# fpthink/PDGN

Hardware: AMD Instinct MI355X
Metric: generator+D step points/sec (B=35, 256->2048 pts) (higher is better)
Workload: dtype f32; 1 GPU; PDGNet_v2 G+D iteration (models/PDGNet_v2.py:171-256), chair-shaped synthetic batch, per-GPU batch 35, 256->2048 pts, random-init weights; global_batch=35, parallelism=dp1, losses_finite=True, hipgraph=False, issue=list

## Files before the change

### pdgn_amd/csrc/gemm_rp.hip

```cpp
#include "gemm_shared.h"

typedef _Float16 rp_f16x8 __attribute__((ext_vector_type(8)));
typedef _Float16 rp_f16x2 __attribute__((ext_vector_type(2)));
typedef float rp_f32x16 __attribute__((ext_vector_type(16)));
typedef float rp_f32x2 __attribute__((ext_vector_type(2)));

struct RpArgs {
    long long M;
    int N, lda, ldw, ldc;
    const float *A;
    const unsigned short *Wp;
    long long wplane;
    float *C;
    const unsigned *max_w;
    int panels, ctiles;
    int rgroups, cslabs;
    int wg_per_xcd;
    float *stat_part;
};

__device__ __forceinline__ unsigned rp_cvt_pk(float a, float b) {
    const rp_f32x2 v = {a, b};
    return __builtin_bit_cast(unsigned, __builtin_convertvector(v, rp_f16x2));
}
__device__ __forceinline__ rp_f32x16 rp_mfma(const u32x4 a, const u32x4 b, const rp_f32x16 c) {
    return __builtin_amdgcn_mfma_f32_32x32x16_f16(__builtin_bit_cast(rp_f16x8, a), __builtin_bit_cast(rp_f16x8, b), c, 0, 0, 0);
}
__device__ __forceinline__ unsigned rp_sw(unsigned r) { return (r >> 2) & 3u; }

template <int K, int AUX, bool PIPE, bool STATS = false>
__global__ __launch_bounds__(512, 1) void gemm_rp_kernel(const RpArgs p) {
    static_assert(K == 32 || K == 64 || K == 128, "reduction lengths of the per-point products");
    constexpr int KS = K / 16, KC = K / 32;
    constexpr int BN = 64, BM = 256;
    constexpr int PLANE = KC * BN * 64;
    constexpr int WTILE = 2 * PLANE;
    constexpr int STL = STATS ? 2 * (8 * 3 * BN + 8) * 4 : 0;
    __shared__ __attribute__((aligned(1024))) unsigned char smem[2 * WTILE + 2 * BN * 4 + 8 * 4096 + STL];
    int *const colexp = reinterpret_cast<int *>(smem + 2 * WTILE);
    float *const stl = reinterpret_cast<float *>(smem + 2 * WTILE + 2 * BN * 4 + 8 * 4096);
    const int tid = threadIdx.x, lane = tid & 63;
    const int wave = __builtin_amdgcn_readfirstlane(tid >> 6);
    unsigned char *const stg = smem + 2 * WTILE + 2 * BN * 4 + wave * 4096;
    const int li = lane & 31, lg = lane >> 5;

    const int xcd = blockIdx.x & 7, slot = blockIdx.x >> 3;
    const int rgi = xcd / p.cslabs, csi = xcd - rgi * p.cslabs;
    const int ppg = (p.panels + p.rgroups - 1) / p.rgroups, cps = (p.ctiles + p.cslabs - 1) / p.cslabs;
    const int p0 = rgi * ppg, p1 = min(p.panels, p0 + ppg);
    const int c0 = csi * cps, c1 = min(p.ctiles, c0 + cps);
    if (p0 >= p1 || c0 >= c1) return;
    const int nc = c1 - c0;
    const long long steps = (long long)(p1 - p0) * nc;
    long long t = steps * slot / p.wg_per_xcd;
    const long long t1 = steps * (slot + 1) / p.wg_per_xcd;
    if (t >= t1) return;

    constexpr int PIECES = 2 * BN * (K / 8) / 512;
    static_assert(PIECES >= 1, "a weight tile is at least one piece per thread");
    u32x4 wraw[PIECES];
    int craw = 0;
    const __amdgpu_buffer_rsrc_t rsW = __builtin_amdgcn_make_buffer_rsrc((void *)p.Wp, 0, (int)min((2 * p.wplane) * 2LL, 0x7fffffffLL), 0x00020000);
    const __amdgpu_buffer_rsrc_t rsMW = __builtin_amdgcn_make_buffer_rsrc((void *)p.max_w, 0, p.N * 4, 0x00020000);
    auto load_w = [&](int ct) {
        const int n0 = (c0 + ct) * BN;
#pragma unroll
        for (int j = 0; j < PIECES; ++j) {
            const int id = tid + 512 * j;
            const int part = id / (BN * (K / 8)), rem = id - part * (BN * (K / 8));
            const int row = rem / (K / 8), c = rem - row * (K / 8);
            const bool ok = ct < nc && n0 + row < p.N;
            const unsigned off = (unsigned)(((long long)part * p.wplane + (long long)(n0 + row) * p.ldw + 8 * c) * 2);
            wraw[j] = __builtin_bit_cast(u32x4, __builtin_amdgcn_raw_buffer_load_b128(rsW, ok ? off : NT_OOB, 0, 0));
        }
        if (tid < BN) craw = __builtin_amdgcn_raw_buffer_load_b32(rsMW, (ct < nc && n0 + tid < p.N) ? (unsigned)(n0 + tid) * 4u : NT_OOB, 0, 0);
    };
    auto write_w = [&](int buf) {
#pragma unroll
        for (int j = 0; j < PIECES; ++j) {
            const int id = tid + 512 * j;
            const int part = id / (BN * (K / 8)), rem = id - part * (BN * (K / 8));
            const int row = rem / (K / 8), c = rem - row * (K / 8);
            *reinterpret_cast<u32x4 *>(smem + buf * WTILE + part * PLANE + (c >> 2) * (BN * 64) + row * 64 + (((c & 3) ^ rp_sw(row)) * 16)) = wraw[j];
        }
        if (tid < BN) colexp[buf * BN + tid] = 127 - x2_scale_field((unsigned)craw);
    };

    u32x4 afh[KS], afl[KS];
    int ua_e[4];
    int cur_mrows = 0;
    __amdgpu_buffer_rsrc_t rsC = __builtin_amdgcn_make_buffer_rsrc((void *)p.C, 0, 0, 0x00020000);
    auto load_a = [&](int panel) {
        const long long m0 = (long long)panel * BM + 32 * wave;
        const int mrows = (int)max(0LL, min(32LL, p.M - m0));
        cur_mrows = mrows;
        const __amdgpu_buffer_rsrc_t rsA = __builtin_amdgcn_make_buffer_rsrc((void *)(p.A + m0 * p.lda), 0,
                                                                            mrows > 0 ? (int)(((long long)(mrows - 1) * p.lda + K) * 4) : 0, 0x00020000);
        f32x4 raw[2 * KS];
#pragma unroll
        for (int s = 0; s < KS; ++s) {
            const unsigned off = li < mrows ? (unsigned)(li * p.lda + 16 * s + 8 * lg) * 4u : NT_OOB;
            raw[2 * s] = __builtin_bit_cast(f32x4, __builtin_amdgcn_raw_buffer_load_b128(rsA, off, 0, 0));
            raw[2 * s + 1] = __builtin_bit_cast(f32x4, __builtin_amdgcn_raw_buffer_load_b128(rsA, off == NT_OOB ? NT_OOB : off + 16u, 0, 0));
        }
        unsigned mb = 0u;
#pragma unroll
        for (int i = 0; i < 2 * KS; ++i)
#pragma unroll
            for (int r = 0; r < 4; ++r) mb = max(mb, __float_as_uint(raw[i][r]) & 0x7fffffffu);
        mb = max(mb, (unsigned)__shfl_xor((int)mb, 32));
        const int f = x2_scale_field(mb);
        const float sc = __int_as_float(f << 23);
#pragma unroll
// ... 171 lines not shown
#pragma unroll
            for (int part = 0; part < 4; ++part) out_part(prev, part);
        }
        const bool more = t + 1 < t1;
        const int nct = next_ct(ct);
        if (more) write_w(buf ^ 1);
        const bool more2 = t + 2 < t1;
        if (more2) load_w(next_ct(nct));
        if (more && nct == 0) {
            ++panel;
            load_a(panel);
        }
        ct = nct;
        buf ^= 1;
        asm volatile("s_waitcnt lgkmcnt(0)" ::: "memory");
        __builtin_amdgcn_s_barrier();
        asm volatile("" ::: "memory");
    }
    if (STATS && comb) stat_combine(comb_panel, comb_n0, comb_sb);
    if (PIPE && have_prev) {
#pragma unroll
        for (int part = 0; part < 4; ++part) out_part(prev, part);
    }
    if (STATS && have_prev) {
        asm volatile("s_waitcnt lgkmcnt(0)" ::: "memory");
        __builtin_amdgcn_s_barrier();
        asm volatile("" ::: "memory");
        stat_combine(prev_panel, prev.n0, prev.sbuf);
    }
}

template <int K>
static void rp_go(int grid, hipStream_t s, const RpArgs &a, int aux, bool pipe) {
    if (a.stat_part) {
        if (aux == 2) hipLaunchKernelGGL((gemm_rp_kernel<K, 2, true, true>), dim3(grid), dim3(512), 0, s, a);
        else hipLaunchKernelGGL((gemm_rp_kernel<K, 0, true, true>), dim3(grid), dim3(512), 0, s, a);
    } else if (!pipe) hipLaunchKernelGGL((gemm_rp_kernel<K, 2, false>), dim3(grid), dim3(512), 0, s, a);
    else if (aux == 16) hipLaunchKernelGGL((gemm_rp_kernel<K, 16, true>), dim3(grid), dim3(512), 0, s, a);
    else if (aux == 2) hipLaunchKernelGGL((gemm_rp_kernel<K, 2, true>), dim3(grid), dim3(512), 0, s, a);
    else hipLaunchKernelGGL((gemm_rp_kernel<K, 0, true>), dim3(grid), dim3(512), 0, s, a);
}

bool rp_takes(long long m, int n, int k) {
    static const bool off = [] { const char *e = getenv("PDGN_RP"); return e && e[0] == '0'; }();
    return !off && (k == 32 || k == 64 || k == 128) && n >= 128 && m >= 4096 && (double)m * n >= 1.6e7 && m < (1LL << 28);
}

int rp_launch(long long m, int n, int k, const float *A, int lda, const unsigned short *Wp, int ldw, long long wplane, float *C, int ldc,
              float *stat_part, hipStream_t s) {
    RpArgs a;
    a.stat_part = stat_part;
    a.M = m; a.N = n; a.lda = lda; a.ldw = ldw; a.ldc = ldc; a.A = A; a.Wp = Wp; a.wplane = wplane; a.C = C;
    a.max_w = reinterpret_cast<const unsigned *>(Wp + 2 * wplane);
    a.panels = cdiv(m, 256);
    a.ctiles = cdiv(n, 64);
    static const int force_cs = [] { const char *e = getenv("PDGN_RP_CSLABS"); return e ? atoi(e) : 0; }();
    int cs = 1;
    while (cs < 8 && (double)cdiv(a.ctiles, cs) * 64 * k * 4 > 2.0e6) cs *= 2;
    if (force_cs == 1 || force_cs == 2 || force_cs == 4 || force_cs == 8) cs = force_cs;
    while (cs > 1 && (a.ctiles < cs || a.panels < 8 / cs)) cs /= 2;
    a.cslabs = cs;
    a.rgroups = 8 / cs;
    const int cus = nt_cus();
    a.wg_per_xcd = cus >= 8 ? cus / 8 : 1;
    static const int aux_env = [] { const char *e = getenv("PDGN_RP_STORE"); return e ? atoi(e) : -1; }();
    const int aux = aux_env >= 0 ? aux_env : ((double)m * n * 4 > 2.5e8 ? 2 : 0);
    static const bool pipe = [] { const char *e = getenv("PDGN_RP_PIPE"); return !(e && e[0] == '0'); }();
    const int grid = 8 * a.wg_per_xcd;
    if (k == 128) rp_go<128>(grid, s, a, aux, pipe);
    else if (k == 64) rp_go<64>(grid, s, a, aux, pipe);
    else rp_go<32>(grid, s, a, aux, pipe);
    return pdgn_launch_status();
}
```

### pdgn_amd/csrc/gemm_x3.hip

```cpp
#include <atomic>
#include <type_traits>

#include "gemm_shared.h"

#ifndef X3_FENCE
#define X3_FENCE 2
#endif
#ifndef X3_DEFAULT_MASK
#define X3_DEFAULT_MASK 0x000
#endif
#ifndef X3_FENCE16
#define X3_FENCE16 2
#endif
#ifndef X3_ABLATE
#define X3_ABLATE 0
#endif

typedef float f32x16 __attribute__((ext_vector_type(16)));
typedef float f32x2 __attribute__((ext_vector_type(2)));
typedef __bf16 bf16x8 __attribute__((ext_vector_type(8)));
typedef __bf16 bf16x2 __attribute__((ext_vector_type(2)));

struct X3Parts {
    u32x4 h, m, l;
// ... 1051 lines not shown
        const unsigned long long at = next.fetch_add(need);
        const unsigned long long pos = at % slots;
        if (pos + need <= slots) return ring + (size_t)pos * 256;
    }
}
const unsigned *x2_scan(const float *X, long long rows, int cols, int ld, bool bycol, hipStream_t s) {
    unsigned *out = x2_arena_take(bycol ? cols : rows);
    if (!out) return nullptr;
    if (x2_maxima_launch(X, rows, cols, ld, bycol ? nullptr : out, bycol ? out : nullptr, s) != 0) return nullptr;
    return out;
}
static thread_local const unsigned *x2_next_max_a = nullptr, *x2_next_max_w = nullptr;

static thread_local const unsigned *x2_cur_max_a = nullptr, *x2_cur_max_w = nullptr;
struct X3Handover {
    X3Handover() {
        x3_cur_ws = x3_tail_ws; x3_cur_ws_floats = x3_tail_ws_floats;
        x2_cur_max_a = x2_next_max_a; x2_cur_max_w = x2_next_max_w;
        x3_tail_ws = nullptr; x3_tail_ws_floats = 0;
        x2_next_max_a = x2_next_max_w = nullptr;
    }
    ~X3Handover() {
        x3_cur_ws = nullptr; x3_cur_ws_floats = 0;
        x2_cur_max_a = x2_cur_max_w = nullptr;
    }
};

static int x3_reduce_split(int tiles) {
    int y = 8;
    while (tiles * y < 512 && y < 64) y *= 2;
    return y;
}

bool rp_takes(long long m, int n, int k);
int rp_launch(long long m, int n, int k, const float *A, int lda, const unsigned short *Wp, int ldw, long long wplane, float *C, int ldc,
              float *stat_part, hipStream_t s);
void x3_launch16(int cfg, int flags, int grid, hipStream_t s, const NtArgs &a);
void x3_launch_h2(int flags, int grid, hipStream_t s, const NtArgs &a, bool eight_waves);
const void *x3_symbol_h2(int flags, bool eight_waves);
static bool x2_pays(int cfg, long long m, int n, int k, long long scan_bytes) {
    if (nt_switches().mode != 2 || cfg != 0 || k < 128 || m >= (1LL << 28)) return false;
    const double flops = 2.0 * (double)m * n * k;
    static const double min_flops = [] { const char *e = getenv("PDGN_X2_MIN_GFLOP"); return (e && *e) ? atof(e) * 1e9 : 2e10; }();
    return flops >= min_flops && (double)scan_bytes <= 4.5e-3 * flops;
}

template <int TM, int TN, int WM, int WN, int OCC, int RATE, int CFG>
struct X3Cfg {
    static constexpr int BM = 32 * TM * WM, BN = 32 * TN * WN;
    static constexpr int LDS = 2 * 3 * (BM + BN) * 64;
    static constexpr int WG_PER_CU = OCC;

    struct Plan {
        int tiles_m, tiles_n, kchunks, grid_dp, dp_tiles, grid_sk;
        long long sk_per_wg;
        double cost;
    };
    static int dp_grid(long long tiles, int slots, int kc) {
        int tpw = (64 + kc - 1) / kc;
        tpw = tpw < 1 ? 1 : (tpw > 8 ? 8 : tpw);
        const long long g = (tiles + tpw - 1) / tpw;
        const long long lo = tiles < slots ? tiles : slots;
        return (int)(g < lo ? lo : g);
    }
    static double chunk_us(int w) { return 2.0 * BM * BN * NT_BK * w / (RATE * 1e3); }
    static Plan plan(long long m, int n, int k, bool allow_sk) {
        Plan pl;
// ... 303 lines not shown

extern "C" int pdgn_gemm_nt_ex(long long m, int n, int k, const float *A, int lda, const float *W, int ldw, const float *bias,
                               const float *addend, int ldadd, float *C, int ldc, float *stat_part, const float *row_bias,
                               int ld_rb, int rows_per_group, int act, const float *gate, int ldgate, int transposed_w,
                               pdgn_stream_t stream) {
    const X3Handover handover;
    if (!x3_mode())
        return fp32_gemm_nt_ex(m, n, k, A, lda, W, ldw, bias, addend, ldadd, C, ldc, stat_part, row_bias, ld_rb, rows_per_group,
                               act, gate, ldgate, transposed_w, stream);
    if (!x3_args_ok(m, n, k, lda, ldw, ldadd, ldc, addend, transposed_w != 0)) return PDGN_ERR_INVALID;
    if ((act != 0 && act != 2) || (row_bias && (ld_rb < n || ld_rb % 4 || rows_per_group < 1)) ||
        (gate && (ldgate < n || ldgate % 4)) || m >= (1LL << 31) || (row_bias && m * rows_per_group >= (1LL << 32)) ||
        (row_bias && rows_per_group >= 1 && ((m + rows_per_group - 1) / rows_per_group) * (long long)ld_rb * 4 >= (long long)NT_OOB))
        return PDGN_ERR_INVALID;
    NtEpi e;
    e.row_bias = row_bias; e.ld_rb = ld_rb; e.rows_per_group = rows_per_group; e.act = act; e.gate = gate; e.ldgate = ldgate;
    return transposed_w ? x3_dispatch<true>(m, n, k, A, lda, W, ldw, bias, addend, ldadd, C, ldc, stat_part, (hipStream_t)stream, e)
                        : x3_dispatch<false>(m, n, k, A, lda, W, ldw, bias, addend, ldadd, C, ldc, stat_part, (hipStream_t)stream, e);
}

extern "C" int pdgn_gemm_nt_ps(long long m, int n, int k, const float *A, int lda, const unsigned short *Wplanes, int ldw,
                               long long wplane, int parts, const float *bias, const float *addend, int ldadd, float *C, int ldc,
                               float *stat_part, const float *row_bias, int ld_rb, int rows_per_group, int act, const float *gate,
                               int ldgate, pdgn_stream_t stream) {
    const X3Handover handover;
    if (!x3_mode() || !Wplanes || (parts != 3 && parts != 2)) return PDGN_ERR_INVALID;
    if (!x3_args_ok(m, n, k, lda, ldw, ldadd, ldc, addend, false)) return PDGN_ERR_INVALID;
    if (wplane < (long long)(n - 1) * ldw + k || wplane >= (1LL << 28) || ldw % 8 || wplane % 8 || ((uintptr_t)Wplanes & 15))
        return PDGN_ERR_INVALID;
    if ((act != 0 && act != 2) || (row_bias && (ld_rb < n || ld_rb % 4 || rows_per_group < 1)) ||
        (gate && (ldgate < n || ldgate % 4)) || m >= (1LL << 31) || (row_bias && m * rows_per_group >= (1LL << 32)) ||
        (row_bias && rows_per_group >= 1 && ((m + rows_per_group - 1) / rows_per_group) * (long long)ld_rb * 4 >= (long long)NT_OOB))
        return PDGN_ERR_INVALID;
    if (parts == 2 && x3_mode() == 2 && !bias && !addend && !row_bias && !act && !gate && rp_takes(m, n, k)) {
        return rp_launch(m, n, k, A, lda, Wplanes, ldw, wplane, C, ldc, stat_part, (hipStream_t)stream);
    }
    NtEpi e;
    e.row_bias = row_bias; e.ld_rb = ld_rb; e.rows_per_group = rows_per_group > 0 ? rows_per_group : 1; e.act = act; e.gate = gate;
    e.ldgate = ldgate;
    return x3_dispatch<false>(m, n, k, A, lda, nullptr, ldw, bias, addend, ldadd, C, ldc, stat_part, (hipStream_t)stream, e, Wplanes,
                              wplane, parts);
}

extern "C" long long pdgn_gemm_tail_workspace_floats(long long m, int n, int k, int with_stats) {
    if (!x3_mode() || m < 1 || n < 4 || k < 4) return 0;
    const bool sk = !with_stats;
    switch (x3_pick(m, n, k, with_stats != 0)) {
        case 0: return X3Big::tail_floats(m, n, k, sk);
        case 2: return X3Narrow::tail_floats(m, n, k, sk);
        default: return X3Square::tail_floats(m, n, k, sk);
    }
}
extern "C" long long pdgn_gemm_nt_ps_workspace_floats(long long m, int n, int k, int parts, int with_stats) {
    if (!x3_mode() || m < 1 || n < 4 || k < 4) return 0;
    if (parts == 2 && rp_takes(m, n, k)) return 0;
    if (parts == 2) return with_stats ? 0 : X3Big::tail_floats(m, n, k, true);
    return pdgn_gemm_tail_workspace_floats(m, n, k, with_stats);
}
extern "C" int pdgn_gemm_set_tail_workspace(float *ws, long long floats) {
    if (floats < 0 || ((uintptr_t)ws & 15)) return PDGN_ERR_INVALID;
    x3_tail_ws = ws;
    x3_tail_ws_floats = ws ? floats : 0;
    return 0;
}

extern "C" int pdgn_gemm_nt_ps_launch_info(long long m, int n, int k, int parts, const void **sym, int *grid) {
    if (!x3_mode() || m < 1 || n < 4 || k < 4 || !sym || !grid) return PDGN_ERR_INVALID;
    const int cfg = x3_pick(m, n, k, false);
    const bool s16 = x3_shape16(cfg, false, false, true);
    *sym = nullptr;
    if (parts == 2) {
        *grid = X3Big::plan(m, n, k, true).grid_dp;
        *sym = x3_symbol_h2(16, true);
    } else if (cfg == 0) {
        *grid = X3Big::plan(m, n, k, true).grid_dp;
        if (!s16) *sym = (const void *)gemm_x3_kernel<4, 2, 2, 2, 1, false, false, false, false, true, 32>;
    } else if (cfg == 2) {
        *grid = X3Narrow::plan(m, n, k, true).grid_dp;
        if (!s16) *sym = (const void *)gemm_x3_kernel<2, 1, 2, 2, 2, false, false, false, false, true, 32>;
    } else {
        *grid = X3Square::plan(m, n, k, true).grid_dp;
        if (!s16) *sym = (const void *)gemm_x3_kernel<2, 2, 2, 2, 1, false, false, false, false, true, 32>;
    }
    return 0;
}

extern "C" int pdgn_gemm_aux_symbols(const void **reduce, const void **scan) {
    if (reduce) *reduce = (const void *)x3_sk_reduce_kernel;
    if (scan) *scan = (const void *)x2_maxima_kernel<8>;
    return 0;
}

extern "C" int pdgn_gemm_tn_big(long long m, int n, int k, const float *dY, int ldy, const float *X, int ldx, float *dW,
                                int dw_is_zero, pdgn_stream_t stream) {
    const X3Handover handover;
    if (!x3_mode()) return fp32_gemm_tn_big(m, n, k, dY, ldy, X, ldx, dW, stream);
    if (m < 1 || n < 4 || k < 4 || n % 4 || k % 4 || ldy % 4 || ldx % 4 || ldy < n || ldx < k || ldy >= (1 << 19) ||
        ldx >= (1 << 19) || m > 0x7fffffffLL * 16)
        return PDGN_ERR_INVALID;
    hipStream_t s = (hipStream_t)stream;
    const int cfg = x3_pick(n, k, (int)(m > 0x7fffffff ? 0x7fffffff : m), false);
    switch (cfg) {
        case 0: return X3Big::launch<true, true>(n, k, (int)m, dY, ldy, X, ldx, nullptr, nullptr, 0, dW, k, nullptr, s, NtEpi(), dw_is_zero != 0);
        case 2: return X3Narrow::launch<true, true>(n, k, (int)m, dY, ldy, X, ldx, nullptr, nullptr, 0, dW, k, nullptr, s, NtEpi(), dw_is_zero != 0);
        default: return X3Square::launch<true, true>(n, k, (int)m, dY, ldy, X, ldx, nullptr, nullptr, 0, dW, k, nullptr, s, NtEpi(), dw_is_zero != 0);
    }
}

extern "C" long long pdgn_gemm_tn_big_workspace_floats(long long m, int n, int k) {
    if (!x3_mode() || m < 1 || n < 4 || k < 4) return 0;
    const int red = (int)(m > 0x7fffffff ? 0x7fffffff : m);
    switch (x3_pick(n, k, red, false)) {
        case 0: return X3Big::at_floats(n, k, red);
        case 2: return X3Narrow::at_floats(n, k, red);
        default: return X3Square::at_floats(n, k, red);
    }
}

extern "C" int pdgn_gemm_nt_ps_row_panel(long long m, int n, int k, int parts, int plain) {
    return (x3_mode() == 2 && parts == 2 && plain && m >= 1 && rp_takes(m, n, k)) ? 1 : 0;
}
extern "C" long long pdgn_gemm_nt_ps_stat_rows(long long m, int n, int k, int parts, int plain) {
    if (x3_mode() == 2 && parts == 2 && plain && m >= 1 && rp_takes(m, n, k)) return (m + 255) / 256;
    return pdgn_gemm_nt_stat_rows(m, n, k);
}
extern "C" int pdgn_gemm_nt_ps_stat_block_rows(long long m, int n, int k, int parts, int plain) {
    if (x3_mode() == 2 && parts == 2 && plain && m >= 1 && rp_takes(m, n, k)) return 256;
    return pdgn_gemm_nt_stat_block_rows(m, n, k);
}

extern "C" long long pdgn_gemm_nt_stat_rows(long long m, int n, int k) {
    if (!x3_mode()) return fp32_gemm_nt_stat_rows(m, n, k);
    if (m < 1 || n < 1 || k < 1) return PDGN_ERR_INVALID;
    switch (x3_pick(m, n, k, true)) {
        case 0: return (long long)cdiv(m, X3Big::BM) * 2;
        case 2: return (long long)cdiv(m, X3Narrow::BM) * 2;
        default: return (long long)cdiv(m, X3Square::BM) * 2;
    }
}

extern "C" int pdgn_gemm_nt_stat_block_rows(long long m, int n, int k) {
    if (!x3_mode()) return fp32_gemm_nt_stat_block_rows(m, n, k);
    if (m < 1 || n < 1 || k < 1) return PDGN_ERR_INVALID;
    switch (x3_pick(m, n, k, true)) {
        case 0: return X3Big::BM / 2;
        case 2: return X3Narrow::BM / 2;
        default: return X3Square::BM / 2;
    }
}

extern "C" int pdgn_gemm_nt_config(long long m, int n, int k, int with_stats) {
    if (!x3_mode()) return fp32_gemm_nt_config(m, n, k, with_stats);
    if (m < 1 || n < 1 || k < 1) return PDGN_ERR_INVALID;
    const int c = x3_pick(m, n, k, with_stats != 0);
    const bool sk = !with_stats;
    const int g = c == 0 ? X3Big::plan(m, n, k, sk).grid_sk : c == 1 ? X3Square::plan(m, n, k, sk).grid_sk
                                                                      : X3Narrow::plan(m, n, k, sk).grid_sk;
    return c + (g ? 16 : 0);
}
#endif
// ... 1 lines not shown
```

### pdgn_amd/fused.py

```python
import os
import weakref

import torch
from ._fn import Function

from . import _lib
from ._lib import check, ptr, require, stream_of

F32 = torch.float32
ACT = {"none": 0, "relu": 1, "leaky_relu": 2}


def _scratch_floats(L, rows, C):
    n = L.pdgn_bn_scratch_floats(rows, C)
    if n < 0:
        raise _lib.PdgnHipError("pdgn_bn_scratch_floats: argument outside the supported range")
    return n


_ZERO_COLSUM = {}


def mark_zero_colsum(dx):
    _ZERO_COLSUM[dx.data_ptr()] = weakref.ref(dx)
# ... 248 lines not shown
    if c % mult == 0 and t.stride(1) == 1 and t.stride(0) % 4 == 0 and t.data_ptr() % 16 == 0:
        return t
    if c % mult == 0:
        return t.contiguous()
    return torch.nn.functional.pad(t, (0, mult - c % mult)).contiguous()


GEMM_LOG = None


_PLANES = os.environ.get("PDGN_PLANES", "1") == "1"


class Planes:
    __slots__ = ("p", "t", "shape", "parts_p", "parts_t")

    def __init__(self, p, t, shape, parts_p=3, parts_t=3):
        self.p, self.t, self.shape, self.parts_p, self.parts_t = p, t, shape, parts_p, parts_t


def two_part(m, n, k, scan_bytes):
    return _lib.gemm_mode() == "x2" and bool(_lib.lib().pdgn_gemm_two_part(m, n, k, scan_bytes))


def two_part_planes(m, n, k, scan_bytes):
    return _lib.gemm_mode() == "x2" and bool(_lib.lib().pdgn_gemm_two_part_planes(m, n, k, scan_bytes))


def _slots(t):
    if _lib.gemm_mode() == "x2":
        _lib.ensure_scale_slots(t.device)


def split_planes(w, want_t, rows=None, dy_maxima_free=False, x_maxima_free=False):
    _slots(w)
    mode = _lib.gemm_mode()
    if (not (_PLANES and w.is_cuda and w.dim() == 2 and mode != "fp32") or w.shape[0] % 4 or w.shape[1] % 4 or w.stride(1) != 1
            or w.stride(0) % 4 or w.data_ptr() % 16):
        return None
    n, k = w.shape
    ldp, ldt = (k + 7) // 8 * 8, (n + 7) // 8 * 8
    parts_p = 2 if rows and two_part_planes(rows, n, k, 0 if x_maxima_free else rows * k * 4) else 3
    parts_t = 2 if rows and want_t and two_part_planes(rows, k, n, 0 if dy_maxima_free else rows * n * 4) else 3

    def planes(parts, rows_, ld):
        buf = torch.empty(parts * rows_ * ld + 2 * rows_ + 8, dtype=torch.int16, device=w.device)
        return buf[:parts * rows_ * ld].view(parts, rows_, ld)
    P = planes(parts_p, n, ldp)
    PT = planes(parts_t, k, ldt) if want_t else None
    L = _lib.lib()
    st = stream_of(w)
    if parts_p == parts_t or not want_t:
        fn = L.pdgn_split_bf16x3 if parts_p == 3 else L.pdgn_split_f16x2
        check(fn(n, k, ptr(w), w.stride(0), ptr(P), ldp, n * ldp, ptr(PT), ldt, k * ldt if want_t else 0, st), "pdgn_split")
    else:
        for parts, args in ((parts_p, (ptr(P), ldp, n * ldp, None, 0, 0)),
                            (parts_t, (None, 0, 0, ptr(PT), ldt, k * ldt))):
            fn = L.pdgn_split_bf16x3 if parts == 3 else L.pdgn_split_f16x2
            check(fn(n, k, ptr(w), w.stride(0), *args, st), "pdgn_split")
    return Planes(P, PT, (n, k), parts_p, parts_t)


def _maxima_ok(t):
    return (_lib.gemm_mode() == "x2" and t.is_cuda and t.dim() == 2 and t.stride(1) == 1 and t.dtype == F32 and t.shape[1] % 4 == 0
            and t.stride(0) % 4 == 0 and t.data_ptr() % 16 == 0)


def operand_maxima(t, rows=True, cols=False):
    if not _maxima_ok(t) or not (rows or cols):
        return (None, None) if (rows and cols) else None
    rm = torch.empty((t.shape[0],), dtype=torch.int32, device=t.device) if rows else None
    cm = torch.empty((t.shape[1],), dtype=torch.int32, device=t.device) if cols else None
    check(_lib.lib().pdgn_absmax_rows_cols(t.shape[0], t.shape[1], ptr(t), t.stride(0), ptr(rm), ptr(cm), stream_of(t)), "pdgn_absmax_rows_cols")
    return (rm, cm) if (rows and cols) else (rm if rows else cm)


def row_maxima_buffer(rows, device):
    return torch.empty((rows,), dtype=torch.int32, device=device)


def _hand_maxima(L, ma, mw=None):
    if ma is not None or mw is not None:
        L.pdgn_gemm_set_operand_scales(ptr(ma), ptr(mw))


def _tail_workspace(L, m, n, k, with_stats, device, parts=None):
    if parts is not None:
        need = L.pdgn_gemm_nt_ps_workspace_floats(m, n, k, parts, 1 if with_stats else 0)
    else:
        need = L.pdgn_gemm_tail_workspace_floats(m, n, k, 1 if with_stats else 0)
    if need <= 0:
        return None
    ws = torch.empty(need, dtype=F32, device=device)
    check(L.pdgn_gemm_set_tail_workspace(ptr(ws), need), "pdgn_gemm_set_tail_workspace")
    return ws


def _rp_takes(m, n, k, parts, plain):
    return parts == 2 and plain and _lib.lib().pdgn_gemm_nt_ps_row_panel(m, n, k, 2, 1) == 1


def planes_fit(P, m, n, k, with_stats=False, plain=False):
    return (P.shape[0] == 3 or not with_stats or _rp_takes(m, n, k, P.shape[0], plain) or (_lib.lib().pdgn_gemm_nt_config(m, n, k, 1) & 15) == 0)


def gemm_nt_planes(a, P, n, k, bias=None, addend=None, want_stats=False, max_a=None):
    _slots(a)
    m = a.shape[0]
    if GEMM_LOG is not None:
        GEMM_LOG.append(("nt", m, n, k))
    ap = _pad_cols(a)
    L = _lib.lib()
    out = torch.empty((m, n), dtype=F32, device=a.device)
    part = None
    if want_stats:
        part = torch.empty((L.pdgn_gemm_nt_ps_stat_rows(m, n, k, P.shape[0], 1 if (bias is None and addend is None) else 0),
                            3 * n), dtype=F32, device=a.device)
    b = bias.detach().contiguous() if bias is not None else None
    if addend is not None:
        addend = _pad_cols(addend)
    ws = _tail_workspace(L, m, n, k, want_stats, a.device, parts=P.shape[0])
    _hand_maxima(L, max_a)
    check(L.pdgn_gemm_nt_ps(m, n, k, ptr(ap), ap.stride(0), ptr(P), P.shape[2], P.shape[1] * P.shape[2], P.shape[0],
                            ptr(b), ptr(addend), addend.stride(0) if addend is not None else 0, ptr(out), n, ptr(part), None, 0, 1, 0,
                            None, 0, stream_of(a)), "pdgn_gemm_nt_ps")
    return (out, part) if want_stats else out


def gemm_nt(a, w, bias=None, addend=None, want_stats=False, w_transposed=False, max_a=None):
    _slots(a)
    m, k = a.shape
    n = w.shape[1] if w_transposed else w.shape[0]
    if GEMM_LOG is not None:
        GEMM_LOG.append(("nn" if w_transposed else "nt", m, n, k))
    ap = _pad_cols(a)
    kp = ap.shape[1]
# ... 84 lines not shown
        GEMM_LOG.append(("thin_tn", m, n, k))
    dw = _zeros((n, k), dy.device)
    db = _zeros((n,), dy.device) if want_db else None
    L = _lib.lib()
    if k <= 4:
        check(L.pdgn_thin_tn(m, k, n, ptr(x), x.stride(0), ptr(dy), dy.stride(0), ptr(dw), 1, k, ptr(None), ptr(db), stream_of(dy)), "pdgn_thin_tn")
    else:
        check(L.pdgn_thin_tn(m, n, k, ptr(dy), dy.stride(0), ptr(x), x.stride(0), ptr(dw), k, 1, ptr(db), ptr(None), stream_of(dy)), "pdgn_thin_tn")
    return dw, db


def _planes_taken(x, weight, planes, want_stats, plain):
    return (planes is not None and x.is_cuda and x.shape[0] >= _PLANES_MIN_ROWS and planes.shape == tuple(weight.shape)
            and x.shape[1] == weight.shape[1] and x.shape[1] % 4 == 0
            and planes_fit(planes.p, x.shape[0], weight.shape[0], weight.shape[1], want_stats, plain))


class LinearCL(Function):

    @staticmethod
    def forward(ctx, x, weight, bias, addend, want_stats=False, planes=None, x_max=None, x_cmax=None):
        ctx.save_for_backward(x, weight)
        ctx.set_materialize_grads(False)
        ctx.has_bias = bias is not None
        ctx.has_addend = addend is not None
        ctx.planes_t = None
        ctx.max_x = None
        ctx.max_x_cols = x_cmax
        if _planes_taken(x, weight, planes, want_stats, bias is None and addend is None):
            n, k = weight.shape
            ctx.thin = False
            ctx.planes_t = planes.t
            xm = None
            if planes.parts_p == 2 and not _rp_takes(x.shape[0], n, k, 2, bias is None and addend is None):
                xm = x_max if x_max is not None else operand_maxima(x)
            ctx.max_x = xm
            if want_stats:
                y, part = gemm_nt_planes(x, planes.p, n, k, bias, addend, want_stats=True, max_a=xm)
                ctx.mark_non_differentiable(part)
                return y, part
            return gemm_nt_planes(x, planes.p, n, k, bias, addend, max_a=xm)
        ctx.thin = bool(x.is_cuda and x.shape[0] >= _OWN_MIN_ROWS and addend is None and weight.is_contiguous()
                        and _thin_ok(x, weight.shape[0], weight.shape[1]))
        if ctx.thin:
            n, k = weight.shape
            if want_stats and k <= 4:
                y, part = thin_nt(x, weight, k, 1, n, bias, want_stats=True)
                ctx.mark_non_differentiable(part)
                return y, part
            y = thin_nt(x, weight, k, 1, n, bias)
            return (y, None) if want_stats else y
        if x.is_cuda and x.shape[0] >= _OWN_MIN_ROWS:
            xm = None
            if want_stats and weight.shape[0] % 4 == 0:
                y, part = gemm_nt(x, weight, bias, addend, want_stats=True, max_a=xm)
                ctx.mark_non_differentiable(part)
                return y, part
            y = gemm_nt(x, weight, bias, addend, max_a=xm)
            return (y, None) if want_stats else y
        y = torch.nn.functional.linear(x, weight, bias)
        y = y + addend if addend is not None else y
        return (y, None) if want_stats else y

    @staticmethod
    def backward(ctx, dy, *unused):
        x, weight = ctx.saved_tensors
        if dy is None:
# ... 629 lines not shown
```

### pdgn_amd/generator.py

```python
import torch
import torch.nn as nn
import torch.nn.functional as F

from . import deconv as _deconv
from .deconv import PointDeconv


def _bn_act(x2d, bn, training, act="leaky_relu", pre_bias=None):
    return _deconv.bn_act(x2d, bn, training, act=act, pre_bias=pre_bias)


def _small_seq(seq, x, training):
    return _deconv.small_sequential(seq, x, training)


def _point_max(x):
    from .fused import point_max
    return point_max(x)


def _linear(rows, weight, bias=None):
    return _deconv.linear_cl(rows, weight, bias)


def _linear_stats(rows, weight, training):
    return _deconv.linear_cl(rows, weight, None, None, bool(training))


def _conv1x1_rows(rows, conv):
    return _linear(rows, _deconv._w2d(conv), conv.bias)


def _head_rows(head, x_rows, B, g=None, n_const=0):
    c0 = head[0]
    W = _deconv._w2d(c0)
    if g is not None and x_rows.is_cuda and x_rows.shape[0] >= 1024 and x_rows.shape[1] % 4 == 0 and n_const % 4 == 0:
        from .fused import HeadMLP
        return HeadMLP.apply(x_rows, g, W, c0.bias, _deconv._w2d(head[2]), head[2].bias, _deconv._w2d(head[4]), head[4].bias, B)
    h = _linear(x_rows, W[:, n_const:].contiguous())
    if g is not None:
        M = x_rows.shape[0] // B
        h = (h.view(B, M, -1) + F.linear(g, W[:, :n_const], c0.bias).unsqueeze(1)).view(B * M, -1)
    else:
        h = h + c0.bias
    h = F.leaky_relu(h)
    h = F.leaky_relu(_conv1x1_rows(h, head[2]))
    return _conv1x1_rows(h, head[4])


class BilateralBlock(nn.Module):

    def __init__(self, level, Fin, Fout, num_k=20, softmax=True):
        super().__init__()
        self.level = level
        if level == 1:
            self.upsample_cov = nn.Sequential(PointDeconv(Fin, Fout, num_k // 2, bilateral=False),
                                              nn.BatchNorm1d(Fout), nn.LeakyReLU(inplace=True))
        else:
            self.upsample_cov = PointDeconv(Fin, Fout, num_k // 2, bilateral=True, softmax=softmax)
# ... 104 lines not shown

    def drop_preassembled(self):
        for dec in self._deconvs():
            dec.drop_preassembled()

    def forward_hints(self):
        return [dec.forward_hints() for dec in self._deconvs()]

    def restore_forward_hints(self, hints):
        for dec, h in zip(self._deconvs(), hints):
            dec.restore_forward_hints(h)


class PointDiscriminator(nn.Module):

    WIDTHS = {1: (64, 128, 256), 2: (64, 128, 256, 512), 3: (64, 128, 256, 512), 4: (64, 128, 256, 1024)}
    HIDDEN = {1: (128, 64), 2: (256, 64), 3: (256, 64), 4: (512, 256, 64)}

    def __init__(self, level, num_point=None):
        super().__init__()
        self.level = level
        self.num_point = num_point if num_point is not None else 128 << level
        layers, cin = [], 3
        for w in self.WIDTHS[level]:
            layers += [nn.Conv1d(cin, w, 1), nn.BatchNorm1d(w), nn.LeakyReLU(inplace=True)]
            cin = w
        self.fc1 = nn.Sequential(*layers)
        mlp = []
        for h in self.HIDDEN[level]:
            mlp += [nn.Linear(cin, h), nn.LeakyReLU(inplace=True)]
            cin = h
        mlp.append(nn.Linear(cin, 1))
        self.mlp = nn.Sequential(*mlp)

    def forward(self, x, aug=None):
        B, _, N = x.shape
        h = x.transpose(1, 2).reshape(B * N, 3) if aug is None else aug.rows(x)
        last = len(self.fc1) - 3
        for i in range(0, last, 3):
            y, part = _linear_stats(h, _deconv._w2d(self.fc1[i]), self.training)
            h = _deconv.bn_act(y, self.fc1[i + 1], self.training, pre_bias=self.fc1[i].bias, partials=part)
        w_last = _deconv._w2d(self.fc1[last])
        y, part = _linear_stats(h, w_last, self.training and not _deconv.STATS_MAX)
        pooled = _deconv.bn_act_maxpool(y, self.fc1[last + 1], self.training, B, N, pre_bias=self.fc1[last].bias, partials=part,
                                        dense=_deconv.DenseInput(h, w_last))
        _deconv.flush_bn_counters()
        return _small_seq(self.mlp, pooled, self.training)


def PointDiscriminator_1(num_point=256):
    return PointDiscriminator(1, num_point)


def PointDiscriminator_2(num_point=512):
    return PointDiscriminator(2, num_point)


def PointDiscriminator_3(num_point=1024):
    return PointDiscriminator(3, num_point)


def PointDiscriminator_4(num_point=2048):
    return PointDiscriminator(4, num_point)


def load_reference_state_dict(module, state_dict):
    clean = {(k[len("module."):] if k.startswith("module.") else k): v for k, v in state_dict.items()}
    return module.load_state_dict(clean, strict=True)
```

### pdgn_amd/trainer.py

```python
import contextlib
import os
import warnings

import torch
import torch.distributed as dist
import torch.nn as nn

from . import _lib
from . import fit as _fit
from . import schedule as _schedule
from . import streams as _streams
from .fused import flush_bn_counters, hold_bn_counters, release_zero_arena
from .generator import PointDiscriminator, PointGenerator
from . import losses
from .fit import GUARD_RECORD_FLOATS, GradGuardError
from .losses import LocalPairLoss
from .optim import FlatGrads, GradGuard, LeanAdamStep

PAIRS = ((0, 1), (0, 2), (0, 3), (1, 2), (1, 3), (2, 3))


class DeterminismWarning(UserWarning):
    """The library's deterministic mode is on, but the operation at hand has no fixed-order form yet."""

# ... 269 lines not shown
        return g["G_epoch"]

    def _loss_weights(self, ws):
        w = self._lw.get(ws)
        if w is None:
            w = self._lw[ws] = torch.tensor([1.2, 1.2, 1.2, 1.0, 0.1 * ws], dtype=torch.float32, device=self.device)
        return w

    def _freeze_D(self, frozen):
        params = self.__dict__.get("_d_params")
        if params is None:
            params = self.__dict__["_d_params"] = [p for d in self.D for p in d.parameters()]
        for p in params:
            p.requires_grad_(not frozen)

    def similar_terms(self, clouds, pairs, own=None):
        terms, own = {}, ({} if own is None else own)
        for a, b in pairs:
            if a not in own:
                cl = clouds[a].transpose(1, 2).contiguous()
                own[a] = self.local_pair.stats(cl, cl)
            terms[(a, b)] = self.local_pair(clouds[a], clouds[b], self_stats=own[a])
        return terms

    @staticmethod
    def _sum_terms(terms):
        return torch.stack([terms[p][0] for p in PAIRS] + [terms[p][1] for p in PAIRS]).sum()

    def similar_loss(self, clouds):
        return self._sum_terms(self.similar_terms(clouds, PAIRS))

    def _seg_d(self, st, i):
        D = self.D[i]
        self.gradD[i].begin()
        if self.aug is None:
            lossD = losses.mse_const(D(st["reals"][i]), 1.0, 0.5) + losses.mse_const(D(st["fakes"][i]), 0.0, 0.5)
        else:
            lossD = (losses.mse_const(D(st["reals"][i], self.aug.at(i, "real")), 1.0, 0.5, self._aug_counter(i))
                     + losses.mse_const(D(st["fakes"][i], self.aug.at(i, "fake")), 0.0, 0.5))
        lossD.backward()
        st["out"]["d_loss%d" % (i + 1)] = lossD.detach()

    def _aug_counter(self, i):
        return self.aug.counter(i) if self.aug is not None and self.aug.adaptive is not None else None

    def _seg_d_real(self, st, i):
        D = self.D[i]
        self.gradD[i].begin()
        params = self.gradD[i].params
        loss_r = losses.mse_const(D(st["reals"][i]) if self.aug is None else D(st["reals"][i], self.aug.at(i, "real")), 1.0, 0.5, self._aug_counter(i))
        st["d_half"][i] = (loss_r.detach(), torch.autograd.grad(loss_r, params))

    def _seg_d_fake(self, st, i):
        D = self.D[i]
        fg = self.gradD[i]
        fg.resume()
        loss_f = losses.mse_const(D(st["fakes"][i]) if self.aug is None else D(st["fakes"][i], self.aug.at(i, "fake")), 0.0, 0.5)
        loss_r, g_real = st["d_half"][i]
        st.setdefault("keep", []).append(loss_r)
        g_fake = torch.autograd.grad(loss_f, fg.params)
        torch._foreach_add_(g_real, g_fake)
        for p, g in zip(fg.params, g_real):
            p.grad = g
        st["d_half"][i] = None
        st["out"]["d_loss%d" % (i + 1)] = loss_r + loss_f.detach()

    def _segment(self, st, k):
        if k == 0:
            if self.aug is not None:
                self.aug.tick()
            with torch.no_grad():
                st["fakes"] = self.G(self._z(st, "z1"))
            self._seg_d(st, 0)
        elif k in (1, 2, 3):
            self._stepD[k - 1].step()
            self._seg_d(st, k)
        elif k == 4:
            self._stepD[3].step()
            self.gradG.begin()
            self._freeze_D(True)
            gen = self.G(self._z(st, "z2"))
            similar = self.similar_loss(gen)
            g_loss = [losses.mse_const(self.D[i](gen[i]) if self.aug is None else self.D[i](gen[i], self.aug.at(i, "gen")), 1.0) for i in range(4)]
            adv = 1.2 * g_loss[0] + 1.2 * g_loss[1] + 1.2 * g_loss[2] + g_loss[3]
            lossG = adv + 0.1 * similar
            ws = st["ws"]
            (adv + (0.1 * ws) * similar if ws > 1 else lossG).backward()
            self._freeze_D(False)
            st["out"]["g_loss"], st["out"]["similar_loss"] = lossG.detach(), similar.detach()
        else:
            self._stepG.step()

    def _z(self, st, name):
        z = st[name]
        return z if z is not None else torch.randn(st["B"], 128, device=self.device) * 0.2

    def _comm(self, k):
        if self.distributed and k < 5:
            fg = self.gradD[k] if k < 4 else self.gradG
            fg.pack()
            fg.all_reduce_mean()

    def _state(self, reals, z1, z2):
        B = reals[0].shape[0]
        return {"reals": reals, "z1": z1, "z2": z2, "B": B, "out": {}, "ws": world_size() if self.distributed else 1}

    def step(self, reals, z1, z2):
        _warn_if_deterministic("step")
        if self.overlap:
            return self._step_overlapped(reals, z1, z2)
        st = self._state(reals, z1, z2)
        for k in range(6):
            self._segment(st, k)
            self._comm(k)
        release_zero_arena()
        return st["out"]

    def _step_overlapped(self, reals, z1, z2, st=None):
        held_counts = hold_bn_counters(True)
        try:
            return self._step_overlapped_body(reals, z1, z2, st)
        finally:
            hold_bn_counters(held_counts)
            flush_bn_counters()
# ... 8 lines not shown
        mark = st.get("mark") or (lambda name: None)
        mark("start")
        if st.get("tag_streams"):
            from . import replay as _replay
            _replay.mark(_replay.MAIN, main)
        if self.aug is not None:
            self.aug.tick()
        if st.get("tag_streams"):
            for sid, s in enumerate(list(pl.d) + [pl.lp, pl.knn], 1):
                s.wait_stream(main)
                _replay.mark(sid, s)

        levels = []

        def d_mark(level, cloud):
            st["fakes"][level] = cloud
            ev = torch.cuda.Event()
            ev.record(torch.cuda.current_stream(self.device))
            levels.append((level, ev))
            if level < 3:
                mark("G(z1) level %d" % (level + 1))

        split = self._split_d

        def d_update(level, ev):
            side = self._side[level]
            side.wait_event(ev)
            with torch.cuda.stream(side), torch.enable_grad():
                if split:
                    self._seg_d_fake(st, level)
                else:
                    self._seg_d(st, level)
                self._comm(level)
                self._stepD[level].step()

        pre_ok = hasattr(self.G, "preassemble") and os.environ.get("PDGN_PREASM", "1") == "1"
        if pre_ok:
            with torch.enable_grad():
                self.G.preassemble(deepest_without_graph=self.distributed and self._buckets)
        if split:
            st["d_half"] = [None] * 4
            for level, side in enumerate(self._side):
                side.wait_stream(main)
                with torch.cuda.stream(side), torch.enable_grad():
                    self._seg_d_real(st, level)

        def d_now(level, cloud):
            d_mark(level, cloud)
            d_update(*levels.pop())

        hook1 = d_mark if self._defer_d else d_now
        with torch.no_grad():
            self.G(self._z(st, "z1"), stage_hook=hook1)
        for level, ev in levels:
            d_update(level, ev)
        mark("G(z1) level 4")
        self.gradG.begin()
        self._freeze_D(True)
        terms, own, g_loss, gen_so_far = {}, {}, [None] * 4, []
        early = self._early_tail

        def d_gen(level, cloud):
            side = self._side[level]
            side.wait_stream(main)
            with torch.cuda.stream(side):
                g_loss[level] = losses.mse_const(self.D[level](cloud) if self.aug is None else self.D[level](cloud, self.aug.at(level, "gen")), 1.0)

# ... 203 lines not shown
```

Measured before the change: 3.138 million points/s.

## Extend row-panel GEMM to K=256 and cache discriminator weight planes

Adds a K=256 variant of the row-panel f16x2 MFMA GEMM. It uses a four-wave workgroup with 128-row panels so the weight tile still fits in LDS, and it is limited to the non-statistics path. The discriminator now caches the split f16 weight planes for each layer and refreshes them in place after each optimizer step. This avoids resplitting the weights on every forward and lets wide K=256 layers take the faster row-panel kernel. The cost is added cache-invalidation logic tied to weight version, pointer and gemm mode, which could go stale if weights change outside these hooks.

Measured after the change: 3.122 million points/s. About the same (-0.5%).

```diff
diff --git a/pdgn_amd/csrc/gemm_rp.hip b/pdgn_amd/csrc/gemm_rp.hip
--- a/pdgn_amd/csrc/gemm_rp.hip
+++ b/pdgn_amd/csrc/gemm_rp.hip
@@ -28,17 +28,24 @@
 }
 __device__ __forceinline__ unsigned rp_sw(unsigned r) { return (r >> 2) & 3u; }
 
+template <int K>
+struct RpShape {
+    static constexpr int WAVES = K == 256 ? 4 : 8, NT = 64 * WAVES, BM = 32 * WAVES;
+};
+
 template <int K, int AUX, bool PIPE, bool STATS = false>
-__global__ __launch_bounds__(512, 1) void gemm_rp_kernel(const RpArgs p) {
-    static_assert(K == 32 || K == 64 || K == 128, "reduction lengths of the per-point products");
+__global__ __launch_bounds__(RpShape<K>::NT, 1) void gemm_rp_kernel(const RpArgs p) {
+    static_assert(K == 32 || K == 64 || K == 128 || K == 256, "reduction lengths of the per-point products");
+    static_assert(!STATS || K <= 128, "the statistics form joins eight waves' sums: not built for the four-wave workgroup");
     constexpr int KS = K / 16, KC = K / 32;
-    constexpr int BN = 64, BM = 256;
+    constexpr int WAVES = RpShape<K>::WAVES, NT = RpShape<K>::NT;
+    constexpr int BN = 64, BM = RpShape<K>::BM;
     constexpr int PLANE = KC * BN * 64;
     constexpr int WTILE = 2 * PLANE;
     constexpr int STL = STATS ? 2 * (8 * 3 * BN + 8) * 4 : 0;
-    __shared__ __attribute__((aligned(1024))) unsigned char smem[2 * WTILE + 2 * BN * 4 + 8 * 4096 + STL];
+    __shared__ __attribute__((aligned(1024))) unsigned char smem[2 * WTILE + 2 * BN * 4 + WAVES * 4096 + STL];
     int *const colexp = reinterpret_cast<int *>(smem + 2 * WTILE);
-    float *const stl = reinterpret_cast<float *>(smem + 2 * WTILE + 2 * BN * 4 + 8 * 4096);
+    float *const stl = reinterpret_cast<float *>(smem + 2 * WTILE + 2 * BN * 4 + WAVES * 4096);
     const int tid = threadIdx.x, lane = tid & 63;
     const int wave = __builtin_amdgcn_readfirstlane(tid >> 6);
     unsigned char *const stg = smem + 2 * WTILE + 2 * BN * 4 + wave * 4096;
@@ -56,7 +63,7 @@
     const long long t1 = steps * (slot + 1) / p.wg_per_xcd;
     if (t >= t1) return;
 
-    constexpr int PIECES = 2 * BN * (K / 8) / 512;
+    constexpr int PIECES = 2 * BN * (K / 8) / NT;
     static_assert(PIECES >= 1, "a weight tile is at least one piece per thread");
     u32x4 wraw[PIECES];
     int craw = 0;
@@ -66,7 +73,7 @@
         const int n0 = (c0 + ct) * BN;
 #pragma unroll
         for (int j = 0; j < PIECES; ++j) {
-            const int id = tid + 512 * j;
+            const int id = tid + NT * j;
             const int part = id / (BN * (K / 8)), rem = id - part * (BN * (K / 8));
             const int row = rem / (K / 8), c = rem - row * (K / 8);
             const bool ok = ct < nc && n0 + row < p.N;
@@ -78,7 +85,7 @@
     auto write_w = [&](int buf) {
 #pragma unroll
         for (int j = 0; j < PIECES; ++j) {
-            const int id = tid + 512 * j;
+            const int id = tid + NT * j;
             const int part = id / (BN * (K / 8)), rem = id - part * (BN * (K / 8));
             const int row = rem / (K / 8), c = rem - row * (K / 8);
             *reinterpret_cast<u32x4 *>(smem + buf * WTILE + part * PLANE + (c >> 2) * (BN * 64) + row * 64 + (((c & 3) ^ rp_sw(row)) * 16)) = wraw[j];
@@ -316,27 +323,35 @@
 
 template <int K>
 static void rp_go(int grid, hipStream_t s, const RpArgs &a, int aux, bool pipe) {
-    if (a.stat_part) {
-        if (aux == 2) hipLaunchKernelGGL((gemm_rp_kernel<K, 2, true, true>), dim3(grid), dim3(512), 0, s, a);
-        else hipLaunchKernelGGL((gemm_rp_kernel<K, 0, true, true>), dim3(grid), dim3(512), 0, s, a);
-    } else if (!pipe) hipLaunchKernelGGL((gemm_rp_kernel<K, 2, false>), dim3(grid), dim3(512), 0, s, a);
-    else if (aux == 16) hipLaunchKernelGGL((gemm_rp_kernel<K, 16, true>), dim3(grid), dim3(512), 0, s, a);
-    else if (aux == 2) hipLaunchKernelGGL((gemm_rp_kernel<K, 2, true>), dim3(grid), dim3(512), 0, s, a);
-    else hipLaunchKernelGGL((gemm_rp_kernel<K, 0, true>), dim3(grid), dim3(512), 0, s, a);
-}
-
-bool rp_takes(long long m, int n, int k) {
+    const dim3 nt(RpShape<K>::NT);
+    if constexpr (K <= 128) {
+        if (a.stat_part) {
+            if (aux == 2) hipLaunchKernelGGL((gemm_rp_kernel<K, 2, true, true>), dim3(grid), nt, 0, s, a);
+            else hipLaunchKernelGGL((gemm_rp_kernel<K, 0, true, true>), dim3(grid), nt, 0, s, a);
+            return;
+        }
+    }
+    if (!pipe) hipLaunchKernelGGL((gemm_rp_kernel<K, 2, false>), dim3(grid), nt, 0, s, a);
+    else if (aux == 16) hipLaunchKernelGGL((gemm_rp_kernel<K, 16, true>), dim3(grid), nt, 0, s, a);
+    else if (aux == 2) hipLaunchKernelGGL((gemm_rp_kernel<K, 2, true>), dim3(grid), nt, 0, s, a);
+    else hipLaunchKernelGGL((gemm_rp_kernel<K, 0, true>), dim3(grid), nt, 0, s, a);
+}
+
+bool rp_takes(long long m, int n, int k, bool stats) {
     static const bool off = [] { const char *e = getenv("PDGN_RP"); return e && e[0] == '0'; }();
-    return !off && (k == 32 || k == 64 || k == 128) && n >= 128 && m >= 4096 && (double)m * n >= 1.6e7 && m < (1LL << 28);
+    static const bool off256 = [] { const char *e = getenv("PDGN_RP_K256"); return e && e[0] == '0'; }();
+    const bool kok = k == 32 || k == 64 || k == 128 || (k == 256 && !stats && !off256);
+    return !off && kok && n >= 128 && m >= 4096 && (double)m * n >= (k == 256 ? 3.0e7 : 1.6e7) && m < (1LL << 28);
 }
 
 int rp_launch(long long m, int n, int k, const float *A, int lda, const unsigned short *Wp, int ldw, long long wplane, float *C, int ldc,
               float *stat_part, hipStream_t s) {
+    if (stat_part && k > 128) return PDGN_ERR_INVALID;
     RpArgs a;
     a.stat_part = stat_part;
     a.M = m; a.N = n; a.lda = lda; a.ldw = ldw; a.ldc = ldc; a.A = A; a.Wp = Wp; a.wplane = wplane; a.C = C;
     a.max_w = reinterpret_cast<const unsigned *>(Wp + 2 * wplane);
-    a.panels = cdiv(m, 256);
+    a.panels = cdiv(m, k == 256 ? RpShape<256>::BM : RpShape<128>::BM);
     a.ctiles = cdiv(n, 64);
     static const int force_cs = [] { const char *e = getenv("PDGN_RP_CSLABS"); return e ? atoi(e) : 0; }();
     int cs = 1;
@@ -351,7 +366,8 @@
     const int aux = aux_env >= 0 ? aux_env : ((double)m * n * 4 > 2.5e8 ? 2 : 0);
     static const bool pipe = [] { const char *e = getenv("PDGN_RP_PIPE"); return !(e && e[0] == '0'); }();
     const int grid = 8 * a.wg_per_xcd;
-    if (k == 128) rp_go<128>(grid, s, a, aux, pipe);
+    if (k == 256) rp_go<256>(grid, s, a, aux, pipe);
+    else if (k == 128) rp_go<128>(grid, s, a, aux, pipe);
     else if (k == 64) rp_go<64>(grid, s, a, aux, pipe);
     else rp_go<32>(grid, s, a, aux, pipe);
     return pdgn_launch_status();
diff --git a/pdgn_amd/csrc/gemm_x3.hip b/pdgn_amd/csrc/gemm_x3.hip
--- a/pdgn_amd/csrc/gemm_x3.hip
+++ b/pdgn_amd/csrc/gemm_x3.hip
@@ -1107,7 +1107,7 @@
     return y;
 }
 
-bool rp_takes(long long m, int n, int k);
+bool rp_takes(long long m, int n, int k, bool stats);
 int rp_launch(long long m, int n, int k, const float *A, int lda, const unsigned short *Wp, int ldw, long long wplane, float *C, int ldc,
               float *stat_part, hipStream_t s);
 void x3_launch16(int cfg, int flags, int grid, hipStream_t s, const NtArgs &a);
@@ -1477,7 +1477,7 @@
         (gate && (ldgate < n || ldgate % 4)) || m >= (1LL << 31) || (row_bias && m * rows_per_group >= (1LL << 32)) ||
         (row_bias && rows_per_group >= 1 && ((m + rows_per_group - 1) / rows_per_group) * (long long)ld_rb * 4 >= (long long)NT_OOB))
         return PDGN_ERR_INVALID;
-    if (parts == 2 && x3_mode() == 2 && !bias && !addend && !row_bias && !act && !gate && rp_takes(m, n, k)) {
+    if (parts == 2 && x3_mode() == 2 && !bias && !addend && !row_bias && !act && !gate && rp_takes(m, n, k, stat_part != nullptr)) {
         return rp_launch(m, n, k, A, lda, Wplanes, ldw, wplane, C, ldc, stat_part, (hipStream_t)stream);
     }
     NtEpi e;
@@ -1498,7 +1498,7 @@
 }
 extern "C" long long pdgn_gemm_nt_ps_workspace_floats(long long m, int n, int k, int parts, int with_stats) {
     if (!x3_mode() || m < 1 || n < 4 || k < 4) return 0;
-    if (parts == 2 && rp_takes(m, n, k)) return 0;
+    if (parts == 2 && rp_takes(m, n, k, with_stats != 0)) return 0;
     if (parts == 2) return with_stats ? 0 : X3Big::tail_floats(m, n, k, true);
     return pdgn_gemm_tail_workspace_floats(m, n, k, with_stats);
 }
@@ -1563,14 +1563,14 @@
 }
 
 extern "C" int pdgn_gemm_nt_ps_row_panel(long long m, int n, int k, int parts, int plain) {
-    return (x3_mode() == 2 && parts == 2 && plain && m >= 1 && rp_takes(m, n, k)) ? 1 : 0;
+    return (x3_mode() == 2 && parts == 2 && (plain & 1) && m >= 1 && rp_takes(m, n, k, (plain & 2) != 0)) ? 1 : 0;
 }
 extern "C" long long pdgn_gemm_nt_ps_stat_rows(long long m, int n, int k, int parts, int plain) {
-    if (x3_mode() == 2 && parts == 2 && plain && m >= 1 && rp_takes(m, n, k)) return (m + 255) / 256;
+    if (x3_mode() == 2 && parts == 2 && plain && m >= 1 && rp_takes(m, n, k, true)) return (m + 255) / 256;
     return pdgn_gemm_nt_stat_rows(m, n, k);
 }
 extern "C" int pdgn_gemm_nt_ps_stat_block_rows(long long m, int n, int k, int parts, int plain) {
-    if (x3_mode() == 2 && parts == 2 && plain && m >= 1 && rp_takes(m, n, k)) return 256;
+    if (x3_mode() == 2 && parts == 2 && plain && m >= 1 && rp_takes(m, n, k, true)) return 256;
     return pdgn_gemm_nt_stat_block_rows(m, n, k);
 }
 
diff --git a/pdgn_amd/fused.py b/pdgn_amd/fused.py
--- a/pdgn_amd/fused.py
+++ b/pdgn_amd/fused.py
@@ -304,7 +304,7 @@
         _lib.ensure_scale_slots(t.device)
 
 
-def split_planes(w, want_t, rows=None, dy_maxima_free=False, x_maxima_free=False):
+def split_planes(w, want_t, rows=None, dy_maxima_free=False, x_maxima_free=False, into=None):
     _slots(w)
     mode = _lib.gemm_mode()
     if (not (_PLANES and w.is_cuda and w.dim() == 2 and mode != "fp32") or w.shape[0] % 4 or w.shape[1] % 4 or w.stride(1) != 1
@@ -318,8 +318,13 @@
     def planes(parts, rows_, ld):
         buf = torch.empty(parts * rows_ * ld + 2 * rows_ + 8, dtype=torch.int16, device=w.device)
         return buf[:parts * rows_ * ld].view(parts, rows_, ld)
-    P = planes(parts_p, n, ldp)
-    PT = planes(parts_t, k, ldt) if want_t else None
+    if (into is not None and into.shape == (n, k) and into.parts_p == parts_p and into.p.device == w.device
+            and (into.t is not None) == bool(want_t) and (not want_t or into.parts_t == parts_t)):
+        P, PT = into.p, into.t
+    else:
+        into = None
+        P = planes(parts_p, n, ldp)
+        PT = planes(parts_t, k, ldt) if want_t else None
     L = _lib.lib()
     st = stream_of(w)
     if parts_p == parts_t or not want_t:
@@ -330,7 +335,7 @@
                             (parts_t, (None, 0, 0, ptr(PT), ldt, k * ldt))):
             fn = L.pdgn_split_bf16x3 if parts == 3 else L.pdgn_split_f16x2
             check(fn(n, k, ptr(w), w.stride(0), *args, st), "pdgn_split")
-    return Planes(P, PT, (n, k), parts_p, parts_t)
+    return into if into is not None else Planes(P, PT, (n, k), parts_p, parts_t)
 
 
 def _maxima_ok(t):
@@ -368,12 +373,12 @@
     return ws
 
 
-def _rp_takes(m, n, k, parts, plain):
-    return parts == 2 and plain and _lib.lib().pdgn_gemm_nt_ps_row_panel(m, n, k, 2, 1) == 1
+def _rp_takes(m, n, k, parts, plain, with_stats=False):
+    return parts == 2 and plain and _lib.lib().pdgn_gemm_nt_ps_row_panel(m, n, k, 2, 3 if with_stats else 1) == 1
 
 
 def planes_fit(P, m, n, k, with_stats=False, plain=False):
-    return (P.shape[0] == 3 or not with_stats or _rp_takes(m, n, k, P.shape[0], plain) or (_lib.lib().pdgn_gemm_nt_config(m, n, k, 1) & 15) == 0)
+    return (P.shape[0] == 3 or not with_stats or _rp_takes(m, n, k, P.shape[0], plain, True) or (_lib.lib().pdgn_gemm_nt_config(m, n, k, 1) & 15) == 0)
 
 
 def gemm_nt_planes(a, P, n, k, bias=None, addend=None, want_stats=False, max_a=None):
@@ -524,7 +529,7 @@
             ctx.thin = False
             ctx.planes_t = planes.t
             xm = None
-            if planes.parts_p == 2 and not _rp_takes(x.shape[0], n, k, 2, bias is None and addend is None):
+            if planes.parts_p == 2 and not _rp_takes(x.shape[0], n, k, 2, bias is None and addend is None, bool(want_stats)):
                 xm = x_max if x_max is not None else operand_maxima(x)
             ctx.max_x = xm
             if want_stats:
diff --git a/pdgn_amd/generator.py b/pdgn_amd/generator.py
--- a/pdgn_amd/generator.py
+++ b/pdgn_amd/generator.py
@@ -4,6 +4,7 @@
 
 from . import deconv as _deconv
 from .deconv import PointDeconv
+from .fused import _PLANES_MIN_ROWS
 
 
 def _bn_act(x2d, bn, training, act="leaky_relu", pre_bias=None):
@@ -23,8 +24,10 @@
     return _deconv.linear_cl(rows, weight, bias)
 
 
-def _linear_stats(rows, weight, training):
-    return _deconv.linear_cl(rows, weight, None, None, bool(training))
+def _linear_stats(rows, weight, training, planes=None):
+    if planes is None:
+        return _deconv.linear_cl(rows, weight, None, None, bool(training))
+    return _deconv.linear_cl(rows, weight, None, None, bool(training), planes)
 
 
 def _conv1x1_rows(rows, conv):
@@ -195,16 +198,44 @@
             cin = h
         mlp.append(nn.Linear(cin, 1))
         self.mlp = nn.Sequential(*mlp)
+        self._planes = {}
+
+    PLANES_MIN_N = 256
+
+    def layer_planes(self, i, weight, rows):
+        if not (weight.is_cuda and weight.dtype == torch.float32 and weight.shape[0] >= self.PLANES_MIN_N and rows >= _PLANES_MIN_ROWS):
+            return None
+        key = (rows, weight.data_ptr(), weight._version, _deconv._lib.gemm_mode())
+        ent = self._planes.get(i)
+        if ent is not None and ent[0] == key:
+            return ent[1]
+        with torch.no_grad():
+            pl = _deconv.split_planes(weight.detach(), False, rows, into=ent[1] if ent is not None else None)
+        self._planes[i] = (key, pl)
+        return pl
+
+    def refresh_planes(self):
+        for i, (key, pl) in list(self._planes.items()):
+            if pl is None:
+                continue
+            weight = _deconv._w2d(self.fc1[i])
+            if key[1] != weight.data_ptr() or key[3] != _deconv._lib.gemm_mode():
+                del self._planes[i]
+                continue
+            with torch.no_grad():
+                new = _deconv.split_planes(weight.detach(), False, key[0], into=pl)
+            self._planes[i] = ((key[0], key[1], weight._version, key[3]), new)
 
     def forward(self, x, aug=None):
         B, _, N = x.shape
         h = x.transpose(1, 2).reshape(B * N, 3) if aug is None else aug.rows(x)
         last = len(self.fc1) - 3
         for i in range(0, last, 3):
-            y, part = _linear_stats(h, _deconv._w2d(self.fc1[i]), self.training)
+            w = _deconv._w2d(self.fc1[i])
+            y, part = _linear_stats(h, w, self.training, self.layer_planes(i, w, h.shape[0]))
             h = _deconv.bn_act(y, self.fc1[i + 1], self.training, pre_bias=self.fc1[i].bias, partials=part)
         w_last = _deconv._w2d(self.fc1[last])
-        y, part = _linear_stats(h, w_last, self.training and not _deconv.STATS_MAX)
+        y, part = _linear_stats(h, w_last, self.training and not _deconv.STATS_MAX, self.layer_planes(last, w_last, h.shape[0]))
         pooled = _deconv.bn_act_maxpool(y, self.fc1[last + 1], self.training, B, N, pre_bias=self.fc1[last].bias, partials=part,
                                         dense=_deconv.DenseInput(h, w_last))
         _deconv.flush_bn_counters()
diff --git a/pdgn_amd/trainer.py b/pdgn_amd/trainer.py
--- a/pdgn_amd/trainer.py
+++ b/pdgn_amd/trainer.py
@@ -325,6 +325,7 @@
 
     def _seg_d(self, st, i):
         D = self.D[i]
+        self._planes_d(i)
         self.gradD[i].begin()
         if self.aug is None:
             lossD = losses.mse_const(D(st["reals"][i]), 1.0, 0.5) + losses.mse_const(D(st["fakes"][i]), 0.0, 0.5)
@@ -339,6 +340,7 @@
 
     def _seg_d_real(self, st, i):
         D = self.D[i]
+        self._planes_d(i)
         self.gradD[i].begin()
         params = self.gradD[i].params
         loss_r = losses.mse_const(D(st["reals"][i]) if self.aug is None else D(st["reals"][i], self.aug.at(i, "real")), 1.0, 0.5, self._aug_counter(i))
@@ -366,10 +368,10 @@
                 st["fakes"] = self.G(self._z(st, "z1"))
             self._seg_d(st, 0)
         elif k in (1, 2, 3):
-            self._stepD[k - 1].step()
+            self._step_d(k - 1)
             self._seg_d(st, k)
         elif k == 4:
-            self._stepD[3].step()
+            self._step_d(3)
             self.gradG.begin()
             self._freeze_D(True)
             gen = self.G(self._z(st, "z2"))
@@ -383,6 +385,17 @@
             st["out"]["g_loss"], st["out"]["similar_loss"] = lossG.detach(), similar.detach()
         else:
             self._stepG.step()
+
+    def _planes_d(self, i):
+        D = self.D[i]
+        if getattr(D, "_planes", None) and torch.cuda.is_current_stream_capturing():
+            D.refresh_planes()
+
+    def _step_d(self, i):
+        self._stepD[i].step()
+        refresh = getattr(self.D[i], "refresh_planes", None)
+        if refresh is not None:
+            refresh()
 
     def _z(self, st, name):
         z = st[name]
@@ -457,7 +470,7 @@
                 else:
                     self._seg_d(st, level)
                 self._comm(level)
-                self._stepD[level].step()
+                self._step_d(level)
 
         pre_ok = hasattr(self.G, "preassemble") and os.environ.get("PDGN_PREASM", "1") == "1"
         if pre_ok:
```
